# mmp/pbrt-v1

Hardware: AMD Instinct MI355X
Metric: Mrays/s (primary+secondary: every Scene::Intersect + Scene::IntersectP) (higher is better)
Workload: dtype f32

## Files before the change

pbrt-v1_amd/csrc/hip/rt_integrate.h:

```cpp
#pragma once
#include "rt_shade.h"
#include "rt_texture.h"
#include "rt_fixed_frame.h"
#include "rt_ray_guard.h"

namespace rt {

enum Stage {
    ST_FETCH = 0, ST_VERTEX, ST_DIRECT_NEXT, ST_SHADOW_DONE, ST_MIS_DONE, ST_ED_BSDF, ST_ED_DONE,
    ST_BOUNCE, ST_SPECULAR, ST_SPEC_TRANS, ST_RETURN, ST_VOL_BEGIN, ST_VOL_STEP, ST_POP, ST_FINISH, ST_EXIT
};

struct Rng {
    uint32_t base, ctr;
    RT_DEV float next_float() { return rng_f32(base, ctr++); }
    RT_DEV uint32_t next_u32() { return rng_u32(base, ctr++); }
};

#define RT_FRAME_WORDS 25

struct Lane {
    uint32_t sample_index;
    uint32_t work;
    float image_x, image_y;
// ... 358 lines not shown
    }
    const int nx = sc.dens_n[0], ny = sc.dens_n[1], nz = sc.dens_n[2];
    const float voxx = (q.x - v.p0[0]) / (v.p1[0] - v.p0[0]) * float(nx) - .5f;
    const float voxy = (q.y - v.p0[1]) / (v.p1[1] - v.p0[1]) * float(ny) - .5f;
    const float voxz = (q.z - v.p0[2]) / (v.p1[2] - v.p0[2]) * float(nz) - .5f;
    const int vx = int(floorf(voxx)), vy = int(floorf(voxy)), vz = int(floorf(voxz));
    const float dx = voxx - float(vx), dy = voxy - float(vy), dz = voxz - float(vz);
    const int x0 = clamp_ref(vx, 0, nx - 1), x1 = clamp_ref(vx + 1, 0, nx - 1);
    const int y0 = clamp_ref(vy, 0, ny - 1), y1 = clamp_ref(vy + 1, 0, ny - 1);
    const int z0 = clamp_ref(vz, 0, nz - 1), z1 = clamp_ref(vz + 1, 0, nz - 1);
    const float RT_G *g = RT_GPTR(const float, sc.dens_grid);
    const int r00 = z0 * nx * ny + y0 * nx, r10 = z0 * nx * ny + y1 * nx, r01 = z1 * nx * ny + y0 * nx, r11 = z1 * nx * ny + y1 * nx;
    const float c000 = g[r00 + x0], c100 = g[r00 + x1], c010 = g[r10 + x0], c110 = g[r10 + x1];
    const float c001 = g[r01 + x0], c101 = g[r01 + x1], c011 = g[r11 + x0], c111 = g[r11 + x1];
    const float d00 = lerp_ref(dx, c000, c100), d10 = lerp_ref(dx, c010, c110);
    const float d01 = lerp_ref(dx, c001, c101), d11 = lerp_ref(dx, c011, c111);
    const float d0 = lerp_ref(dy, d00, d10), d1 = lerp_ref(dy, d01, d11);
    return lerp_ref(dz, d0, d1);
}
RT_DEV V3 density_tau(const DevScene &sc, const DevFrame &fr, V3 o, V3 d, float mint, float maxt, float step, float u) {
    const float length = len3(d);
    if (length == 0.f) return mk3(0.f);
    const float inv = 1.f / length;
    const V3 dn = mk3(d.x * inv, d.y * inv, d.z * inv);
    float t0, t1;
    if (!vol_intersect(sc.vol, o, dn, mint * length, maxt * length, t0, t1)) return mk3(0.f);
    const V3 sig_t = mat_color(sc.vol.sigma_a) + mat_color(sc.vol.sigma_s);
    V3 tau = mk3(0.f);
    t0 += u * step;
    const int cap = fr.dens_cap;
#pragma unroll 1
    for (int k = 0; t0 < t1 && k < cap; ++k) {
        const float D = density_at(sc, xform_point(sc.vol.world_to_volume, o + dn * t0));
        tau = tau + sig_t * D;
        t0 += step;
    }
    return tau * step;
}
RT_DEV V3 exp_neg(V3 tau) { return mk3(rt_expf(-tau.x), rt_expf(-tau.y), rt_expf(-tau.z)); }

template <bool VOL, bool EXT>
RT_DEV V3 scene_transmittance(const DevScene &sc, const DevFrame &fr, Lane &ln, V3 o, V3 d, float mint, float maxt) {
    if (!VOL) return mk3(1.f);
    const float u = ln.rng.next_float();
    if (EXT && sc.dens_kind != RT_DENSITY_NONE) return exp_neg(density_tau(sc, fr, o, d, mint, maxt, 4.f * fr.step_size, u));
    return vol_transmittance(sc.vol, o, d, mint, maxt);
}

template <class SX>
RT_DEV decltype(auto) light_of(const DevScene &sc, int i) {
    if constexpr (SX::one_light) return (RT_LIGHT_K(sc));
    else return (RT_LIGHT(sc, i));
}
template <class SX>
RT_DEV DimReq light_dim(const DevFrame &fr, int li, int k) {
    if constexpr (SX::one_light) { const DimReq r = RT_KPTR(const DimReq, fr.light_dims)[k]; return r; }
    else { const DimReq r = (RT_GPTR(const DimReq, fr.light_dims) + 3 * li)[k]; return r; }
}
template <bool EXT, bool DEFER = false, bool GEOM_N = false, class SX = fixed::AnyScene, int ACCEL = -1>
RT_DEV void estimate_direct_bsdf(const DevScene &sc, Lane &ln) {
    const auto &Lt = light_of<SX>(sc, ln.cur_light);
    ln.stage = ST_ED_DONE;
    if (light_is_delta<EXT>(Lt)) return;
    MatRef m = RT_MAT(sc, ln.v.mat);
    V3 wi; float bsdfPdf; int sampled;
    V3 f = bsdf_sample_f<EXT>(m, ln.v, ln.v.wo, wi, ln.bs1, ln.bs2, ln.bcs, bsdfPdf, BX_ALL & ~BX_SPECULAR, sampled);
    if (!is_black(f) && bsdfPdf > 0.f) {
        float lightPdf;
        if constexpr (EXT) lightPdf = light_is_infinite<EXT>(Lt) ? infinite_pdf_cosine(GEOM_N ? ln.v.ng : ln.v.nn, wi) : area_light_pdf<EXT, SX::one_light>(sc, Lt, ln.v.p, wi);
        else lightPdf = area_light_pdf<EXT, SX::one_light>(sc, Lt, ln.v.p, wi);
        if (lightPdf > 0.f) {
            float fw = 1 * bsdfPdf, gw = 1 * lightPdf;
            float weight = (fw * fw) / (fw * fw + gw * gw);
            ln.pend = div_s(((f * mat_color(Lt.color)) * absdot3(wi, GEOM_N ? ln.v.ng : ln.v.nn)) * weight, bsdfPdf);
            launch_ray<DEFER, ACCEL>(ln, sc, ln.v.p, wi, RT_RAY_EPSILON, RT_INF, false, ST_MIS_DONE);
        }
    }
}

RT_DEV bool light_draws_rng(LightRef L) { return L.type == RT_LIGHT_AREA && L.quadric < 0 && L.n_tris > 1u; }
RT_DEV size_t weighted_record(const DevFrame &fr, const Lane &ln, int nLights) {
    if (!fr.wt_mixed) return size_t(ln.ord) * size_t(1 + 2 * nLights);
    const size_t j = ln.ord - RT_GPTR(const unsigned, fr.wt_base)[ln.work];
    return size_t(RT_GPTR(const unsigned, fr.wt_recbase)[ln.work]) + j * size_t(1 + 2 * (nLights - int(fr.wt_nd))) + size_t(fr.wt_nd) * j * (j + 1);
}

template <bool EXT, bool DEFER = false, bool GEOM_N = false, class SX = fixed::AnyScene, int ACCEL = -1>
RT_DEV void estimate_direct_begin(const DevScene &sc, Lane &ln, int light, float ls1, float ls2) {
    ln.cur_light = light;
    ln.Ld = mk3(0.f);
    const auto &Lt = light_of<SX>(sc, light);
    MatRef m = RT_MAT(sc, ln.v.mat);
    V3 wi, Li, sd; float lightPdf, smax;
    if (light_is_delta<EXT>(Lt)) {
        Li = delta_light_sample(Lt, ln.v.p, wi, sd, smax);
        lightPdf = 1.f;
    } else if constexpr (EXT) {
        if (light_is_infinite<EXT>(Lt)) {
            wi = infinite_sample_cosine(GEOM_N ? ln.v.ng : ln.v.nn, ls1, ls2, ln.rng, lightPdf);
            Li = mat_color(Lt.color);
            sd = wi; smax = RT_INF;
        } else {
            V3 ns;
            V3 ps = area_sample_point<EXT, SX::one_light>(sc, Lt, ln.v.p, ls1, ls2, ln.rng, ns);
            wi = normalize3(ps - ln.v.p);
            lightPdf = area_light_pdf<EXT, SX::one_light>(sc, Lt, ln.v.p, wi);
            Li = area_L(Lt, ns, -wi);
            sd = ps - ln.v.p; smax = 1.f - RT_RAY_EPSILON;
        }
    } else {
        V3 ns;
        V3 ps = area_sample_point<EXT, SX::one_light>(sc, Lt, ln.v.p, ls1, ls2, ln.rng, ns);
        wi = normalize3(ps - ln.v.p);
        lightPdf = area_light_pdf<EXT, SX::one_light>(sc, Lt, ln.v.p, wi);
        Li = area_L(Lt, ns, -wi);
        sd = ps - ln.v.p; smax = 1.f - RT_RAY_EPSILON;
    }
    if (lightPdf > 0.f && !is_black(Li)) {
        V3 f = bsdf_f<EXT>(m, ln.v, ln.v.wo, wi);
        if (!is_black(f)) {
            if (light_is_delta<EXT>(Lt)) ln.pend = div_s((f * Li) * absdot3(wi, GEOM_N ? ln.v.ng : ln.v.nn), lightPdf);
            else {
                float bsdfPdf = bsdf_pdf<EXT>(m, ln.v, ln.v.wo, wi);
                float fw = 1 * lightPdf, gw = 1 * bsdfPdf;
                float weight = (fw * fw) / (fw * fw + gw * gw);
                ln.pend = div_s(((f * Li) * absdot3(wi, GEOM_N ? ln.v.ng : ln.v.nn)) * weight, lightPdf);
            }
            launch_ray<DEFER, ACCEL>(ln, sc, ln.v.p, sd, RT_RAY_EPSILON, smax, true, ST_SHADOW_DONE);
            return;
        }
    }
    ln.stage = ST_ED_BSDF;
}

struct March { int i, N; float t0, step; V3 Tr, p, Lv; float s0, s1, s2; };
template <bool EXT>
RT_DEV void march_begin(const DevScene &sc, const DevFrame &fr, Lane &ln, const Ray &ray, March &m, float RT_G *samp, size_t st) {
    const RtVolume &vol = sc.vol;
    const bool single = fr.volume_integrator == RT_VOLUME_SINGLE;
    int N; float t0, t1, step; V3 p;
    if (!vol_intersect(vol, ray.o, ray.d, ray.mint, ray.maxt, t0, t1) || (t1 - t0) == 0.f) { N = 0; step = 0.f; p = ray.o; }
    else {
        N = int(ceilf((t1 - t0) / fr.step_size));
        step = (t1 - t0) / N;
        p = ray.o + ray.d * t0;
        t0 += dim_value(fr, ln, fr.one_d[fr.n1d - 1], 0, 0) * step;
        if (single) {
            if (N > fr.vol_nmax) { N = fr.vol_nmax; }
            const float delta = 1.f / N;
            for (int a = 0; a < N; ++a) for (int b = 0; b < 3; ++b) samp[size_t(3 * a + b) * st] = (a + ln.rng.next_float()) * delta;
            for (int b = 0; b < 3; ++b) for (int a = 0; a < N; ++a) {
                const int other = int(ln.rng.next_u32() % uint32_t(N));
                const float tmp = samp[size_t(3 * a + b) * st]; samp[size_t(3 * a + b) * st] = samp[size_t(3 * other + b) * st]; samp[size_t(3 * other + b) * st] = tmp;
            }
        }
    }
    m.i = 0; m.N = N; m.t0 = t0; m.step = step; m.Tr = mk3(1.f); m.p = p; m.Lv = mk3(0.f);
    if (EXT && sc.dens_kind != RT_DENSITY_NONE) {
        const V3 T = exp_neg(density_tau(sc, fr, ray.o, ray.d, ray.mint, ray.maxt, fr.step_size, dim_value(fr, ln, fr.one_d[fr.n1d - 2], 0, 0)));
        ln.L = T * ln.L;
    }
}
template <bool COUNT, bool EXT, bool DEFER, bool PREFETCH = false>
RT_DEV bool march_steps(const DevScene &sc, const DevFrame &fr, Lane &ln, const Ray &ray, March &m, const float RT_G *samp, size_t st, bool resume, unsigned *c_any) {
    const RtVolume &vol = sc.vol;
    const bool single = fr.volume_integrator == RT_VOLUME_SINGLE;
    int i = m.i; const int N = m.N; float t0 = m.t0; const float step = m.step; V3 Tr = m.Tr, p = m.p, Lv = m.Lv;
    const V3 w = -ray.d;
    bool have_row = false;
    if (resume) {
        if (COUNT) ++*c_any;
        if (ln.tv.hit_prim < 0)
            Lv = Lv + ln.pend * scene_transmittance<true, EXT>(sc, fr, ln, ln.tv.o, ln.tv.d, ln.tv.mint, ln.tv.maxt);
        ++i; t0 += step;
        have_row = PREFETCH;
    }
// ... 287 lines not shown
        const int nLights = SX::one_light ? 1 : int(sc.n_lights);
        if constexpr (WEIGHTED) {
            if (fr.weighted_phase == 2) {
                const unsigned at = fr.wt_mixed ? __float_as_uint(ln.wt_w) : 1u + 2u * unsigned(ln.li);
                float RT_G *rec = RT_GPTR(float, fr.wt_rec) + weighted_record(fr, ln, nLights) + at;
                rec[0] = lum_y(ln.Ld);
                rec[1] = lum_y(ln.Ld * float(nLights));
                if (fr.wt_mixed) {
                    ln.wt_w = __uint_as_float(at + 2u);
                    const unsigned j = ln.ord - RT_GPTR(const unsigned, fr.wt_base)[ln.work];
                    if (light_draws_rng(RT_LIGHT(sc, ln.li)) && unsigned(ln.lj) < j) ++ln.lj; else { ln.lj = 0; ++ln.li; }
                } else ++ln.li;
                ln.stage = ST_DIRECT_NEXT;
            } else {
                if (ln.wt_w == 0.f) ln.L = ln.L + ln.Ld * float(nLights);
                else ln.L = ln.L + div_s(ln.Ld, ln.wt_w);
                ln.stage = ST_SPECULAR;
            }
            return;
        }
        if (INTEG == RT_INTEGRATOR_PATH) {
            ln.L = ln.L + ln.thr * (ln.Ld * float(nLights));
            ln.stage = ST_BOUNCE;
        } else if (fr.strategy == RT_STRATEGY_ONE) {
            ln.L = ln.L + ln.Ld * float(nLights);
            ln.stage = ST_SPECULAR;
        } else {
            ln.Ld_light = ln.Ld_light + ln.Ld;
            if constexpr (SX::one_light && FX::all_n1) {
                ln.L_all = ln.L_all + ln.Ld_light * (1.f / float(1));
                ln.lj = 0; ln.li = 1;
                all_lights_done(ln);
                return;
            }
            const int ns = FX::all_n1 ? 1 : SX::one_light ? int(RT_KPTR(const DimReq, fr.light_dims)[0].n) : int(RT_GPTR(const DimReq, fr.light_dims)[3 * ln.li].n);
            if (++ln.lj >= ns) {
                ln.L_all = ln.L_all + ln.Ld_light * (1.f / float(ns));
                ln.lj = 0; ++ln.li;
            }
            ln.stage = ST_DIRECT_NEXT;
            if (ln.li >= nLights) all_lights_done(ln);
        }
        return;
    }
    if constexpr (STAGE == ST_BOUNCE) {
        MatRef m = RT_MAT(sc, ln.v.mat);
        const int k = ln.depth;
        float bs1, bs2, bcs;
        if (k < 3) {
            bs1 = dim_value<FX>(fr, ln, fr.two_d[3 * k + 2], 0, 0); bs2 = dim_value<FX>(fr, ln, fr.two_d[3 * k + 2], 0, 1);
            bcs = dim_value<FX>(fr, ln, fr.one_d[3 * k + 2], 0, 0);
        } else { bs1 = ln.rng.next_float(); bs2 = ln.rng.next_float(); bcs = ln.rng.next_float(); }
        V3 wi; float pdf; int flags;
        V3 f = bsdf_sample_f<EXT>(m, ln.v, ln.v.wo, wi, bs1, bs2, bcs, pdf, BX_ALL, flags);
        if (is_black(f) || pdf == 0.f) { ln.stage = ST_RETURN; return; }
        ln.specular = !SX::no_specular && (flags & BX_SPECULAR) != 0;
        ln.thr = ln.thr * div_s(f * absdot3(wi, ln.v.nn), pdf);
        if (k > 3) {
            if (ln.rng.next_float() > .5f) { ln.stage = ST_RETURN; return; }
            ln.thr = div_s(ln.thr, .5f);
        }
        if (k == fr.max_depth) { ln.stage = ST_RETURN; return; }
        ++ln.depth;
        launch_ray<DEFER, ACCEL>(ln, sc, ln.v.p, wi, RT_RAY_EPSILON, RT_INF, false, ST_VERTEX);
        return;
    }
    if constexpr (STAGE == ST_SPECULAR && SX::no_specular) {
        if (!(ln.depth < fr.max_depth)) { ln.stage = ST_RETURN; return; }
        ln.rng.ctr += 3u;
        ln.stage = ST_SPEC_TRANS;
        return;
    } else if constexpr (STAGE == ST_SPEC_TRANS && SX::no_specular) {
        ln.rng.ctr += 3u;
        ln.stage = ST_RETURN;
        return;
    } else if constexpr (STAGE == ST_POP && SX::no_specular && !VOL) {
        ln.stage = ST_FINISH;
        return;
    }
    if constexpr (STAGE == ST_SPECULAR) {
        if (!(ln.depth < fr.max_depth)) { ln.stage = ST_RETURN; return; }
        MatRef m = RT_MAT(sc, ln.v.mat);
        float u3 = ln.rng.next_float(), u2 = ln.rng.next_float(), u1 = ln.rng.next_float();
        V3 wi; float pdf; int flags;
        V3 f = bsdf_sample_f<EXT>(m, ln.v, ln.v.wo, wi, u1, u2, u3, pdf, BX_REFLECTION | BX_SPECULAR, flags);
        if (!is_black(f) && pdf > 0.f) f = div_s(f, pdf);
        const float ad = absdot3(wi, ln.v.nn);
        if (!is_black(f) && ad > 0.f) {
            frame_push<EXT>(fr, ln, gtid, f, ad, ST_SPEC_TRANS);
            ++ln.depth;
            launch_ray<DEFER, ACCEL>(ln, sc, ln.v.p, wi, RT_RAY_EPSILON, RT_INF, false, ST_VERTEX);
            if (VOL) { Ray cr; cr.o = ln.v.p; cr.d = wi; cr.mint = RT_RAY_EPSILON; cr.maxt = RT_INF; vol_store_ray(fr, ln.fsp, gtid, cr); }
            return;
        }
        ln.stage = ST_SPEC_TRANS;
        return;
    }
    if constexpr (STAGE == ST_SPEC_TRANS) {
        MatRef m = RT_MAT(sc, ln.v.mat);
        float u3 = ln.rng.next_float(), u2 = ln.rng.next_float(), u1 = ln.rng.next_float();
        V3 wi; float pdf; int flags;
        V3 f = bsdf_sample_f<EXT>(m, ln.v, ln.v.wo, wi, u1, u2, u3, pdf, BX_TRANSMISSION | BX_SPECULAR, flags);
        if (!is_black(f) && pdf > 0.f) f = div_s(f, pdf);
        const float ad = absdot3(wi, ln.v.nn);
        if (!is_black(f) && ad > 0.f) {
            frame_push<EXT>(fr, ln, gtid, f, ad, ST_RETURN);
            ++ln.depth;
// ... 176 lines not shown
```

pbrt-v1_amd/csrc/hip/rt_shade.h:

```cpp
#pragma once
#include "rt_traverse.h"

namespace rt {

enum { BX_REFLECTION = 1, BX_TRANSMISSION = 2, BX_DIFFUSE = 4, BX_GLOSSY = 8, BX_SPECULAR = 16,
       BX_ALL = 31 };

struct Vertex {
    V3 p, nn, sn, tn;
    V3 ng;
    V3 wo;
    int mat, light;
};

RT_DEV void tri_frame(V3 p1, V3 p2, V3 p3, bool flip, V3 &nn, V3 &dpdu) {
    const float du1 = 0.f - 1.f, du2 = 1.f - 1.f, dv1 = 0.f - 1.f, dv2 = 0.f - 1.f;
    V3 dp1 = p1 - p3, dp2 = p2 - p3;
    const float determinant = du1 * dv2 - dv1 * du2;
    const float invdet = 1.f / determinant;
    dpdu = (dv2 * dp1 - dv1 * dp2) * invdet;
    V3 dpdv = (-du2 * dp1 + du1 * dp2) * invdet;
    nn = normalize3(cross3(dpdu, dpdv));
    if (flip) nn = nn * -1.f;
}
// ... 236 lines not shown
    return p;
}
RT_DEV float diffuse_pdf(V3 wo, V3 wi) { return (wo.z * wi.z > 0.f) ? fabsf(wi.z) * RT_INV_PI : 0.f; }
RT_DEV float glossy_pdf(MatRef m, V3 wo, V3 wi) { return (wo.z * wi.z > 0.f) ? blinn_pdf(m.exponent, wo, wi) : 0.f; }
RT_DEV float diffuse_t_pdf(V3 wo, V3 wi) { return diffuse_pdf(wo, -wi); }
RT_DEV float glossy_t_pdf(MatRef m, V3 wo, V3 wi) { return glossy_pdf(m, wo, -wi); }

template <bool EXT> RT_DEV bool mat_has_diffuse(MatRef m) { return m.type == RT_MAT_MATTE || (EXT && (m.type == RT_MAT_PLASTIC || ((m.type == RT_MAT_UBER || m.type == RT_MAT_TRANSLUCENT) && m.has_r))); }
template <bool EXT> RT_DEV bool mat_has_glossy(MatRef m) { return EXT && (m.type == RT_MAT_PLASTIC || m.type == RT_MAT_SHINYMETAL || ((m.type == RT_MAT_UBER || m.type == RT_MAT_TRANSLUCENT) && m.has_g)); }
template <bool EXT> RT_DEV bool mat_has_diffuse_t(MatRef m) { return EXT && m.type == RT_MAT_TRANSLUCENT && m.has_t; }
template <bool EXT> RT_DEV bool mat_has_glossy_t(MatRef m) { return EXT && m.type == RT_MAT_TRANSLUCENT && m.has_kr; }
RT_DEV bool flags_match(int type, int flags) { return (type & flags) == type; }

template <bool EXT>
RT_DEV int bsdf_num_components(MatRef m, int flags) {
    int n = 0;
    if (EXT && m.type == RT_MAT_UBER) {
        if (m.has_t && flags_match(BX_TRANSMISSION | BX_SPECULAR, flags)) ++n;
        if (m.has_r && flags_match(BX_REFLECTION | BX_DIFFUSE, flags)) ++n;
        if (m.has_g && flags_match(BX_REFLECTION | BX_GLOSSY, flags)) ++n;
        if (m.has_kr && flags_match(BX_REFLECTION | BX_SPECULAR, flags)) ++n;
        return n;
    }
    if (EXT && m.type == RT_MAT_SHINYMETAL) return int(flags_match(BX_REFLECTION | BX_GLOSSY, flags)) + int(flags_match(BX_REFLECTION | BX_SPECULAR, flags));
    if (EXT && m.type == RT_MAT_TRANSLUCENT) {
        if (m.has_r && flags_match(BX_REFLECTION | BX_DIFFUSE, flags)) ++n;
        if (m.has_t && flags_match(BX_TRANSMISSION | BX_DIFFUSE, flags)) ++n;
        if (m.has_g && flags_match(BX_REFLECTION | BX_GLOSSY, flags)) ++n;
        if (m.has_kr && flags_match(BX_TRANSMISSION | BX_GLOSSY, flags)) ++n;
        return n;
    }
    if (m.type == RT_MAT_MATTE || (EXT && m.type == RT_MAT_PLASTIC)) {
        if (((BX_REFLECTION | BX_DIFFUSE) & flags) == (BX_REFLECTION | BX_DIFFUSE)) ++n;
        if (EXT && m.type == RT_MAT_PLASTIC && ((BX_REFLECTION | BX_GLOSSY) & flags) == (BX_REFLECTION | BX_GLOSSY)) ++n;
    } else {
        if (m.has_r && ((BX_REFLECTION | BX_SPECULAR) & flags) == (BX_REFLECTION | BX_SPECULAR)) ++n;
        if (m.type == RT_MAT_GLASS && m.has_t && ((BX_TRANSMISSION | BX_SPECULAR) & flags) == (BX_TRANSMISSION | BX_SPECULAR)) ++n;
    }
    return n;
}
template <bool EXT> RT_DEV int bsdf_total_components(MatRef m) { return bsdf_num_components<EXT>(m, BX_ALL); }

template <bool EXT>
RT_DEV V3 bsdf_f_lobes(MatRef m, V3 wo, V3 wi, int flags) {
    V3 f = mk3(0.f);
    if (mat_has_diffuse<EXT>(m) && flags_match(BX_REFLECTION | BX_DIFFUSE, flags)) f = f + diffuse_f(m, wo, wi);
    if (mat_has_diffuse_t<EXT>(m) && flags_match(BX_TRANSMISSION | BX_DIFFUSE, flags)) f = f + diffuse_t_f(m);
    if (mat_has_glossy<EXT>(m) && flags_match(BX_REFLECTION | BX_GLOSSY, flags)) f = f + microfacet_f(m, wo, wi);
    if (mat_has_glossy_t<EXT>(m) && flags_match(BX_TRANSMISSION | BX_GLOSSY, flags)) f = f + microfacet_t_f(m, wo, wi);
    return f;
}
template <bool EXT> RT_DEV bool mat_has_btdf(MatRef m) { return mat_has_diffuse_t<EXT>(m) || mat_has_glossy_t<EXT>(m); }

template <bool EXT>
RT_DEV V3 bsdf_f(MatRef m, const Vertex &v, V3 woW, V3 wiW) {
    if (!mat_has_diffuse<EXT>(m) && !mat_has_glossy<EXT>(m) && !mat_has_btdf<EXT>(m)) return mk3(0.f);
    V3 wi = to_local(v, wiW), wo = to_local(v, woW);
    if (dot3(wiW, vertex_ng<EXT>(v)) * dot3(woW, vertex_ng<EXT>(v)) > 0) return bsdf_f_lobes<EXT>(m, wo, wi, BX_ALL & ~BX_TRANSMISSION);
    if (mat_has_btdf<EXT>(m)) return bsdf_f_lobes<EXT>(m, wo, wi, BX_ALL & ~BX_REFLECTION);
    return mk3(0.f);
}

template <bool EXT>
RT_DEV float bsdf_pdf(MatRef m, const Vertex &v, V3 woW, V3 wiW) {
    int nc = bsdf_total_components<EXT>(m);
    if (nc == 0) return 0.f;
    if (!mat_has_diffuse<EXT>(m) && !mat_has_glossy<EXT>(m) && !mat_has_btdf<EXT>(m)) return 0.f / float(nc);
    V3 wo = to_local(v, woW), wi = to_local(v, wiW);
    float pdf = 0.f;
    if (mat_has_diffuse<EXT>(m)) pdf += diffuse_pdf(wo, wi);
    if (mat_has_diffuse_t<EXT>(m)) pdf += diffuse_t_pdf(wo, wi);
    if (mat_has_glossy<EXT>(m)) pdf += glossy_pdf(m, wo, wi);
    if (mat_has_glossy_t<EXT>(m)) pdf += glossy_t_pdf(m, wo, wi);
    return pdf / nc;
}

template <bool EXT>
RT_DEV V3 bsdf_f_flags(MatRef m, const Vertex &v, V3 woW, V3 wiW, int flags) {
    const V3 wi = to_local(v, wiW), wo = to_local(v, woW);
    if (dot3(wiW, vertex_ng<EXT>(v)) * dot3(woW, vertex_ng<EXT>(v)) > 0) flags &= ~BX_TRANSMISSION;
    else flags &= ~BX_REFLECTION;
    return bsdf_f_lobes<EXT>(m, wo, wi, flags);
}
template <bool EXT>
RT_DEV float bsdf_pdf_flags(MatRef m, const Vertex &v, V3 woW, V3 wiW, int flags) {
    const int nc = bsdf_num_components<EXT>(m, flags);
    if (nc == 0) return 0.f;
    const V3 wo = to_local(v, woW), wi = to_local(v, wiW);
    float pdf = 0.f;
    if (mat_has_diffuse<EXT>(m) && flags_match(BX_REFLECTION | BX_DIFFUSE, flags)) pdf += diffuse_pdf(wo, wi);
    if (mat_has_diffuse_t<EXT>(m) && flags_match(BX_TRANSMISSION | BX_DIFFUSE, flags)) pdf += diffuse_t_pdf(wo, wi);
    if (mat_has_glossy<EXT>(m) && flags_match(BX_REFLECTION | BX_GLOSSY, flags)) pdf += glossy_pdf(m, wo, wi);
    if (mat_has_glossy_t<EXT>(m) && flags_match(BX_TRANSMISSION | BX_GLOSSY, flags)) pdf += glossy_t_pdf(m, wo, wi);
    return pdf / nc;
}

template <bool EXT>
RT_DEV V3 bsdf_sample_f(MatRef m, const Vertex &v, V3 woW, V3 &wiW, float u1, float u2, float u3,
                        float &pdf, int flags, int &sampled) {
    sampled = 0; pdf = 0.f;
    int matching = bsdf_num_components<EXT>(m, flags);
    if (matching == 0) return mk3(0.f);
    int which = min(int(floorf(u3 * matching)), matching - 1);
    V3 wo = to_local(v, woW);
    V3 wi, f;
    const bool diffuse_has = mat_has_diffuse<EXT>(m) && flags_match(BX_REFLECTION | BX_DIFFUSE, flags);
    const bool glossy_has = mat_has_glossy<EXT>(m) && flags_match(BX_REFLECTION | BX_GLOSSY, flags);
    const bool diffuse_t_has = mat_has_diffuse_t<EXT>(m) && flags_match(BX_TRANSMISSION | BX_DIFFUSE, flags);
    const bool glossy_t_has = mat_has_glossy_t<EXT>(m) && flags_match(BX_TRANSMISSION | BX_GLOSSY, flags);
    const bool shiny = EXT && m.type == RT_MAT_SHINYMETAL;
    int pick = 0;
    if (shiny) {
        int idx = which;
        if (glossy_has && idx-- == 0) pick = 2;
        else if (flags_match(BX_REFLECTION | BX_SPECULAR, flags)) pick = 3;
    } else if (EXT && m.type == RT_MAT_TRANSLUCENT) {
        int idx = which;
        if (diffuse_has && idx-- == 0) pick = 1;
        else if (diffuse_t_has && idx-- == 0) pick = 5;
        else if (glossy_has && idx-- == 0) pick = 2;
        else if (glossy_t_has) pick = 6;
    } else if (EXT && m.type == RT_MAT_UBER) {
        int idx = which;
        const bool mT = m.has_t && flags_match(BX_TRANSMISSION | BX_SPECULAR, flags), mR = m.has_kr && flags_match(BX_REFLECTION | BX_SPECULAR, flags);
        if (mT && idx-- == 0) pick = 4;
        else if (diffuse_has && idx-- == 0) pick = 1;
        else if (glossy_has && idx-- == 0) pick = 2;
        else if (mR) pick = 3;
    } else if (diffuse_has || glossy_has) pick = (!glossy_has || (diffuse_has && which == 0)) ? 1 : 2;
    if (pick == 1 || pick == 2 || (EXT && (pick == 5 || pick == 6))) {
        const bool through = EXT && (pick == 5 || pick == 6);
        if (pick == 1 || (EXT && pick == 5)) {
            float dx, dy; concentric_disk(u1, u2, dx, dy);
            wi = mk3(dx, dy, sqrtf(fmaxf(0.f, 1.f - dx * dx - dy * dy)));
            if (wo.z < 0.f) wi.z *= -1.f;
            pdf = diffuse_pdf(wo, wi);
            if (pdf == 0.f) return mk3(0.f);
            sampled = through ? (BX_TRANSMISSION | BX_DIFFUSE) : (BX_REFLECTION | BX_DIFFUSE);
            if (through) wi = other_hemisphere(wi);
            if (through && diffuse_has) pdf += diffuse_pdf(wo, wi);
            if (!through && diffuse_t_has) pdf += diffuse_t_pdf(wo, wi);
            if (glossy_has) pdf += glossy_pdf(m, wo, wi);
            if (glossy_t_has) pdf += glossy_t_pdf(m, wo, wi);
        } else {
            const float costheta = rt_powf(u1, 1.f / (m.exponent + 1));
            const float sintheta = sqrtf(fmaxf(0.f, 1.f - costheta * costheta));
            const float phi = u2 * 2.f * RT_PI;
            V3 H = mk3(sintheta * rt_cosf(phi), sintheta * rt_sinf(phi), costheta);
            if (!(wo.z * H.z > 0.f)) H = -H;
            wi = -wo + H * (2.f * dot3(wo, H));
            pdf = ((m.exponent + 1.f) * rt_powf(costheta, m.exponent)) / (2.f * RT_PI * 4.f * dot3(wo, H));
            if (dot3(wo, H) <= 0.f) pdf = 0.f;
            if (pdf == 0.f) return mk3(0.f);
// ... 3 lines not shown
            if (diffuse_t_has) pdf += diffuse_t_pdf(wo, wi);
            if (through && glossy_has) pdf += glossy_pdf(m, wo, wi);
            if (!through && glossy_t_has) pdf += glossy_t_pdf(m, wo, wi);
        }
        wiW = to_world(v, wi);
        if (matching > 1) pdf /= matching;
        f = mk3(0.f);
        if (dot3(wiW, vertex_ng<EXT>(v)) * dot3(woW, vertex_ng<EXT>(v)) > 0) f = bsdf_f_lobes<EXT>(m, wo, wi, flags & ~BX_TRANSMISSION);
        else if (mat_has_btdf<EXT>(m)) f = bsdf_f_lobes<EXT>(m, wo, wi, flags & ~BX_REFLECTION);
        return f;
    }
    bool reflect_has = m.has_r && ((BX_REFLECTION | BX_SPECULAR) & flags) == (BX_REFLECTION | BX_SPECULAR);
    bool pick_reflect = ((EXT && m.type == RT_MAT_UBER) || shiny) ? pick == 3 : (reflect_has && which == 0);
    if (pick_reflect) {
        wi = mk3(-wo.x, -wo.y, wo.z);
        pdf = 1.f;
        const bool uber = EXT && m.type == RT_MAT_UBER;
        float F = (m.type == RT_MAT_GLASS) ? fresnel_dielectric(wo.z, 1.f, m.ior) : (uber ? fresnel_dielectric(wo.z, 1.5f, 1.f) : 1.f);
        if (shiny) f = div_s(fr_cond(fabsf(wo.z), mat_color(m.kr)) * mk3(1.f), fabsf(wi.z));
        else f = div_s(mk3(F) * (uber ? mat_color(m.kr) : mat_color(m.r)), fabsf(wi.z));
        sampled = BX_REFLECTION | BX_SPECULAR;
    } else {
        bool entering = wo.z > 0.f;
        float ei = 1.f, et = m.ior;
        if (!entering) { float tmp = ei; ei = et; et = tmp; }
        float sini2 = sin_theta2(wo);
        float eta = ei / et;
        float sint2 = eta * eta * sini2;
        if (sint2 >= 1.f) return mk3(0.f);
        float cost = sqrtf(fmaxf(0.f, 1.f - sint2));
        if (entering) cost = -cost;
        wi = mk3(eta * -wo.x, eta * -wo.y, cost);
        pdf = 1.f;
        float F = fresnel_dielectric(wo.z, 1.f, m.ior);
        f = div_s(((mk3(1.f) - mk3(F)) * ((et * et) / (ei * ei))) * mat_color(m.t), fabsf(wi.z));
        sampled = BX_TRANSMISSION | BX_SPECULAR;
    }
    wiW = to_world(v, wi);
    if (matching > 1) pdf /= matching;
    return f;
}

template <bool K = false>
RT_DEV void light_tri(const DevScene &sc, unsigned k, V3 &p1, V3 &p2, V3 &p3) {
    if constexpr (K) {
        const float RT_K *t = RT_KPTR(const float, sc.light_tris) + size_t(k) * 16;
        p1 = mk3(t[0], t[1], t[2]); p2 = mk3(t[3], t[4], t[5]); p3 = mk3(t[6], t[7], t[8]);
    } else {
    const float RT_G *t = RT_GPTR(const float, sc.light_tris) + size_t(k) * 16;
    p1 = mk3(t[0], t[1], t[2]); p2 = mk3(t[3], t[4], t[5]); p3 = mk3(t[6], t[7], t[8]);
    }
}

template <bool EXT, class LT> RT_DEV bool light_is_infinite(const LT &Lt) { return EXT && Lt.type == RT_LIGHT_INFINITE; }
template <bool EXT, class LT> RT_DEV bool light_is_delta(const LT &Lt) {
    if constexpr (EXT) return Lt.type != RT_LIGHT_AREA && Lt.type != RT_LIGHT_INFINITE;
    else return Lt.type != RT_LIGHT_AREA;
}
template <class LT>
RT_DEV V3 delta_light_sample(const LT &Lt, V3 p, V3 &wi, V3 &sd, float &smax) {
    if (Lt.type == RT_LIGHT_DISTANT) {
        wi = mk3(Lt.dir[0], Lt.dir[1], Lt.dir[2]);
        sd = wi; smax = RT_INF;
        return mat_color(Lt.color);
    }
    const V3 lp = mat_color(Lt.pos);
    const V3 dd = lp - p;
    wi = normalize3(dd);
    sd = dd; smax = 1.f - RT_RAY_EPSILON;
    const float d2 = dd.x * dd.x + dd.y * dd.y + dd.z * dd.z;
    if (Lt.type == RT_LIGHT_POINT) return div_s(mat_color(Lt.color), d2);
    const V3 w = -wi;
    const V3 wl = normalize3(mk3(Lt.w2l[0] * w.x + Lt.w2l[1] * w.y + Lt.w2l[2] * w.z, Lt.w2l[3] * w.x + Lt.w2l[4] * w.y + Lt.w2l[5] * w.z,
                                 Lt.w2l[6] * w.x + Lt.w2l[7] * w.y + Lt.w2l[8] * w.z));
    const float costheta = wl.z;
    float fall;
    if (costheta < Lt.cos_total) fall = 0.f;
    else if (costheta > Lt.cos_falloff) fall = 1.f;
    else { const float delta = (costheta - Lt.cos_total) / (Lt.cos_falloff - Lt.cos_total); fall = delta * delta * delta * delta; }
    return div_s(mat_color(Lt.color) * fall, d2);
}

RT_DEV void coordinate_system(V3 v1, V3 &v2, V3 &v3) {
    if (fabsf(v1.x) > fabsf(v1.y)) { const float il = 1.f / sqrtf(v1.x * v1.x + v1.z * v1.z); v2 = mk3(-v1.z * il, 0.f, v1.x * il); }
    else { const float il = 1.f / sqrtf(v1.y * v1.y + v1.z * v1.z); v2 = mk3(0.f, v1.z * il, -v1.y * il); }
    v3 = cross3(v1, v2);
}
template <class RNG>
RT_DEV V3 infinite_sample_cosine(V3 n, float u1, float u2, RNG &rng, float &pdf) {
    float x, y; concentric_disk(u1, u2, x, y);
    float z = sqrtf(fmaxf(0.f, 1.f - x * x - y * y));
    if (rng.next_float() < .5f) z *= -1.f;
    pdf = fabsf(z) * RT_INV_TWOPI;
    V3 v1, v2; coordinate_system(normalize3(n), v1, v2);
    return mk3(v1.x * x + v2.x * y + n.x * z, v1.y * x + v2.y * y + n.y * z, v1.z * x + v2.z * y + n.z * z);
}
RT_DEV float infinite_pdf_cosine(V3 n, V3 wi) { return absdot3(n, wi) * RT_INV_TWOPI; }
RT_DEV V3 infinite_sample_sphere(float u1, float u2, float &pdf) {
    const float z = 1.f - 2.f * u1;
    const float r = sqrtf(fmaxf(0.f, 1.f - z * z));
    const float phi = 2.f * RT_PI * u2;
    pdf = 1.f / (4.f * RT_PI);
    return mk3(r * rt_cosf(phi), r * rt_sinf(phi), z);
}
RT_DEV V3 infinite_le_sum(const DevScene &sc, V3 acc, V3 w, bool weighted) {
    if (sc.n_infinite == 0) return acc;
// ... 25 lines not shown
        const float r = sqrtf(fmaxf(0.f, 1.f - z * z));
        const float phi = 2.f * RT_PI * u2;
        p = mk3(0.f) + mk3(r * rt_cosf(phi), r * rt_sinf(phi), z) * q.radius;
        n = p;
    }
    ns = normalize3(xform_normal(q.w2o, n));
    if (ro) ns = ns * -1.f;
    return xform_point(q.o2w, p);
}
RT_DEV V3 quadric_sample(const DevScene &sc, unsigned qi, bool ro, V3 p, float u1, float u2, V3 &ns) {
    const DevQuadric RT_G &q = RT_GPTR(const DevQuadric, sc.quadrics)[qi];
    if (q.type != RT_QUADRIC_SPHERE) return quadric_sample_uniform(q, ro, u1, u2, ns);
    const V3 Pcenter = xform_point(q.o2w, mk3(0.f));
    const V3 wc = normalize3(Pcenter - p);
    V3 wcX, wcY;
    if (fabsf(wc.x) > fabsf(wc.y)) { const float il = 1.f / sqrtf(wc.x * wc.x + wc.z * wc.z); wcX = mk3(-wc.z * il, 0.f, wc.x * il); }
    else { const float il = 1.f / sqrtf(wc.y * wc.y + wc.z * wc.z); wcX = mk3(0.f, wc.z * il, -wc.y * il); }
    wcY = cross3(wc, wcX);
    if (dist_sq(p, Pcenter) - q.radius * q.radius < 1e-4f) return quadric_sample_uniform(q, ro, u1, u2, ns);
    const float cosThetaMax = sqrtf(fmaxf(0.f, 1.f - q.radius * q.radius / dist_sq(p, Pcenter)));
    const float costheta = (1.f - u1) * cosThetaMax + u1 * 1.f;
    const float sintheta = sqrtf(1.f - costheta * costheta);
    const float phi = u2 * 2.f * RT_PI;
    const V3 rd = wcX * (rt_cosf(phi) * sintheta) + wcY * (rt_sinf(phi) * sintheta) + wc * costheta;
    float thit;
    if (!quadric_test(sc, qi, p, rd, RT_RAY_EPSILON, RT_INF, thit)) thit = dot3(Pcenter - p, normalize3(rd));
    const V3 ps = p + rd * thit;
    ns = normalize3(ps - Pcenter);
    if (ro) ns = ns * -1.f;
    return ps;
}
RT_DEV float quadric_area(const DevQuadric RT_G &q) {
    return q.type == RT_QUADRIC_DISK ? q.phi_max * 0.5f * (q.radius * q.radius - q.zmax * q.zmax)
                                     : (q.type == RT_QUADRIC_CYLINDER ? (q.zmax - q.zmin) * q.phi_max * q.radius : q.phi_max * q.radius * (q.zmax - q.zmin));
}
RT_DEV float quadric_light_pdf(const DevScene &sc, unsigned qi, V3 p, V3 wi) {
    const DevQuadric RT_G &q = RT_GPTR(const DevQuadric, sc.quadrics)[qi];
    if (q.type == RT_QUADRIC_SPHERE) {
        const V3 Pcenter = xform_point(q.o2w, mk3(0.f));
        if (!(dist_sq(p, Pcenter) - q.radius * q.radius < 1e-4f)) {
            const float cosThetaMax = sqrtf(fmaxf(0.f, 1.f - q.radius * q.radius / dist_sq(p, Pcenter)));
            return 1.f / (2.f * RT_PI * (1.f - cosThetaMax));
        }
    }
    float thit;
    if (!quadric_test(sc, qi, p, wi, RT_RAY_EPSILON, RT_INF, thit)) return 0.f;
    V3 hp, nn, sn; quadric_frame(sc, qi, false, p, wi, thit, hp, nn, sn);
    const float area = quadric_area(q);
    float pdf = dist_sq(p, p + wi * thit) / (absdot3(nn, -wi) * area);
    if (absdot3(nn, -wi) == 0.f) pdf = 0.f;
    return pdf;
}

template <bool EXT, bool K = false, class LT>
RT_DEV float area_light_pdf(const DevScene &sc, const LT &L, V3 p, V3 wi) {
    if (EXT && L.quadric >= 0) return quadric_light_pdf(sc, unsigned(L.quadric), p, wi);
    bool any = false; float thit = 0.f; V3 nl = mk3(0.f);
    for (unsigned k = 0; k < L.n_tris; ++k) {
        V3 p1, p2, p3; light_tri<K>(sc, L.first_tri + k, p1, p2, p3);
        float t, b1, b2;
        if (tri_test(p1, p2 - p1, p3 - p1, p, wi, RT_RAY_EPSILON, RT_INF, t, b1, b2)) {
            any = true; thit = t;
            if constexpr (K) {
                const float RT_K *ltr = RT_KPTR(const float, sc.light_tris) + size_t(L.first_tri + k) * 16;
                nl = mk3(ltr[12], ltr[13], ltr[14]);
            } else {
            const float RT_G *ltr = RT_GPTR(const float, sc.light_tris) + size_t(L.first_tri + k) * 16;
            nl = mk3(ltr[12], ltr[13], ltr[14]);
            }
        }
    }
    if (!any) return 0.f;
    V3 ph = p + wi * thit;
    V3 dd = p - ph;
    float ad = absdot3(nl, -wi);
    float pdf = (dd.x * dd.x + dd.y * dd.y + dd.z * dd.z) / (ad * L.area);
    if (ad == 0.f) pdf = 0.f;
    return pdf;
}

template <class LT> RT_DEV V3 area_L(const LT &L, V3 n, V3 w) { return dot3(n, w) > 0 ? mat_color(L.color) : mk3(0.f); }

template <bool EXT, bool K = false, class LT, class RNG>
RT_DEV V3 area_sample_point(const DevScene &sc, const LT &L, V3 pref, float u1, float u2, RNG &rng, V3 &ns) {
    if (EXT && L.quadric >= 0) return quadric_sample(sc, unsigned(L.quadric), L.reverse_orientation != 0, pref, u1, u2, ns);
    unsigned k = 0;
    if (L.n_tris > 1) {
        float ls = rng.next_float();
        for (k = 0; k < L.n_tris - 1; ++k) {
            if constexpr (K) { if (ls < RT_KPTR(const float, sc.light_tris)[size_t(L.first_tri + k) * 16 + 10]) break; }
            else
            if (ls < RT_GPTR(const float, sc.light_tris)[size_t(L.first_tri + k) * 16 + 10]) break;
        }
    }
    V3 p1, p2, p3; light_tri<K>(sc, L.first_tri + k, p1, p2, p3);
    float su1 = sqrtf(u1);
    float b1 = 1.f - su1, b2 = u2 * su1;
    V3 ps = b1 * p1 + b2 * p2 + (1.f - b1 - b2) * p3;
    ns = normalize3(cross3(p2 - p1, p3 - p1));
    if (L.reverse_orientation) ns = ns * -1.f;
    return ps;
}

RT_DEV V3 uniform_sample_cone(float u1, float u2, float costhetamax) {
    const float costheta = (1.f - u1) * costhetamax + u1 * 1.f;
    const float sintheta = sqrtf(1.f - costheta * costheta);
    const float phi = u2 * 2.f * RT_PI;
    return mk3(rt_cosf(phi) * sintheta, rt_sinf(phi) * sintheta, costheta);
}
RT_DEV V3 light_to_world(LightRef Lt, V3 v) {
    const float inv = Lt.l2w_scale;
    return mk3((Lt.l2w[0] * v.x + Lt.l2w[1] * v.y + Lt.l2w[2] * v.z) * inv, (Lt.l2w[3] * v.x + Lt.l2w[4] * v.y + Lt.l2w[5] * v.z) * inv,
               (Lt.l2w[6] * v.x + Lt.l2w[7] * v.y + Lt.l2w[8] * v.z) * inv);
}
template <bool EXT, class RNG>
RT_DEV void light_sample_emission(const DevScene &sc, LightRef Lt, V3 wc, float wr, float u1, float u2, float u3, float u4, RNG &rng, V3 &o, V3 &d, float &pdf) {
    if (Lt.type == RT_LIGHT_POINT) {
        o = mat_color(Lt.pos);
        d = infinite_sample_sphere(u1, u2, pdf);
    } else if (Lt.type == RT_LIGHT_SPOT) {
        o = mat_color(Lt.pos);
        d = light_to_world(Lt, uniform_sample_cone(u1, u2, Lt.cos_total));
        pdf = 1.f / (2.f * RT_PI * (1.f - Lt.cos_total));
    } else if (Lt.type == RT_LIGHT_DISTANT) {
        const V3 lightDir = mat_color(Lt.dir);
        V3 v1, v2; coordinate_system(lightDir, v1, v2);
        float d1, d2; concentric_disk(u1, u2, d1, d2);
        const V3 Pdisk = wc + wr * (d1 * v1 + d2 * v2);
        o = Pdisk + wr * lightDir;
        d = -lightDir;
        pdf = 1.f / (RT_PI * wr * wr);
    } else if (Lt.type == RT_LIGHT_INFINITE) {
        const float worldRadius = wr * 1.01f;
        float unused;
        const V3 p1 = wc + worldRadius * infinite_sample_sphere(u1, u2, unused);
        const V3 p2 = wc + worldRadius * infinite_sample_sphere(u3, u4, unused);
        o = p1;
        d = normalize3(p2 - p1);
// ... 22 lines not shown
```

Baseline: 3686.

## Specialize direct lighting for single small emitters and matte-only scenes

Adds a fast path for scenes with one light and at most two emitter triangles. Both triangles are loaded from constant memory once and reused for area sampling and the pdf, instead of looping over triangle indices. It also copies the light header into registers and adds a diffuse-only BSDF path (f, pdf, sample) for scenes known to have no specular materials. This cuts redundant loads and lobe dispatch in the shading stage, but raises register pressure and adds more template code paths.

New measurement: 3755 (median of 6 runs). 1.02x the previous value.

```diff
diff --git a/pbrt-v1_amd/csrc/hip/rt_integrate.h b/pbrt-v1_amd/csrc/hip/rt_integrate.h
--- a/pbrt-v1_amd/csrc/hip/rt_integrate.h
+++ b/pbrt-v1_amd/csrc/hip/rt_integrate.h
@@ -434,6 +434,19 @@
     if constexpr (SX::one_light) return (RT_LIGHT_K(sc));
     else return (RT_LIGHT(sc, i));
 }
+#ifndef RT_EMITTER_HOIST
+#define RT_EMITTER_HOIST 1
+#endif
+struct LightHead { int type; float color[3]; unsigned first_tri, n_tris; int reverse_orientation; float area; int quadric; };
+template <class SX, class LT>
+RT_DEV decltype(auto) light_head(const LT &L) {
+    if constexpr (SX::one_light && RT_EMITTER_HOIST != 0) {
+        LightHead h;
+        h.type = L.type; h.color[0] = L.color[0]; h.color[1] = L.color[1]; h.color[2] = L.color[2];
+        h.first_tri = L.first_tri; h.n_tris = L.n_tris; h.reverse_orientation = L.reverse_orientation; h.area = L.area; h.quadric = L.quadric;
+        return h;
+    } else return (L);
+}
 template <class SX>
 RT_DEV DimReq light_dim(const DevFrame &fr, int li, int k) {
     if constexpr (SX::one_light) { const DimReq r = RT_KPTR(const DimReq, fr.light_dims)[k]; return r; }
@@ -441,12 +454,13 @@
 }
 template <bool EXT, bool DEFER = false, bool GEOM_N = false, class SX = fixed::AnyScene, int ACCEL = -1>
 RT_DEV void estimate_direct_bsdf(const DevScene &sc, Lane &ln) {
-    const auto &Lt = light_of<SX>(sc, ln.cur_light);
+    const auto &Ld = light_of<SX>(sc, ln.cur_light);
+    const auto &Lt = light_head<SX>(Ld);
     ln.stage = ST_ED_DONE;
     if (light_is_delta<EXT>(Lt)) return;
     MatRef m = RT_MAT(sc, ln.v.mat);
     V3 wi; float bsdfPdf; int sampled;
-    V3 f = bsdf_sample_f<EXT>(m, ln.v, ln.v.wo, wi, ln.bs1, ln.bs2, ln.bcs, bsdfPdf, BX_ALL & ~BX_SPECULAR, sampled);
+    V3 f = bsdf_sample_f<EXT, SX::no_specular>(m, ln.v, ln.v.wo, wi, ln.bs1, ln.bs2, ln.bcs, bsdfPdf, BX_ALL & ~BX_SPECULAR, sampled);
     if (!is_black(f) && bsdfPdf > 0.f) {
         float lightPdf;
         if constexpr (EXT) lightPdf = light_is_infinite<EXT>(Lt) ? infinite_pdf_cosine(GEOM_N ? ln.v.ng : ln.v.nn, wi) : area_light_pdf<EXT, SX::one_light>(sc, Lt, ln.v.p, wi);
@@ -471,11 +485,12 @@
 RT_DEV void estimate_direct_begin(const DevScene &sc, Lane &ln, int light, float ls1, float ls2) {
     ln.cur_light = light;
     ln.Ld = mk3(0.f);
-    const auto &Lt = light_of<SX>(sc, light);
+    const auto &Ld = light_of<SX>(sc, light);
+    const auto &Lt = light_head<SX>(Ld);
     MatRef m = RT_MAT(sc, ln.v.mat);
     V3 wi, Li, sd; float lightPdf, smax;
     if (light_is_delta<EXT>(Lt)) {
-        Li = delta_light_sample(Lt, ln.v.p, wi, sd, smax);
+        Li = delta_light_sample(Ld, ln.v.p, wi, sd, smax);
         lightPdf = 1.f;
     } else if constexpr (EXT) {
         if (light_is_infinite<EXT>(Lt)) {
@@ -490,6 +505,20 @@
             Li = area_L(Lt, ns, -wi);
             sd = ps - ln.v.p; smax = 1.f - RT_RAY_EPSILON;
         }
+    } else if constexpr (SX::one_light && RT_SMALL_EMITTER != 0) {
+        V3 ns, ps;
+        if (emitter_is_small(Lt)) {
+            const EmitterPair e = emitter_pair(sc, Lt);
+            ps = area_sample_point_small(e, Lt, ls1, ls2, ln.rng, ns);
+            wi = normalize3(ps - ln.v.p);
+            lightPdf = area_light_pdf_small(e, Lt, ln.v.p, wi);
+        } else {
+            ps = area_sample_point<EXT, true, false>(sc, Lt, ln.v.p, ls1, ls2, ln.rng, ns);
+            wi = normalize3(ps - ln.v.p);
+            lightPdf = area_light_pdf<EXT, true, false>(sc, Lt, ln.v.p, wi);
+        }
+        Li = area_L(Lt, ns, -wi);
+        sd = ps - ln.v.p; smax = 1.f - RT_RAY_EPSILON;
     } else {
         V3 ns;
         V3 ps = area_sample_point<EXT, SX::one_light>(sc, Lt, ln.v.p, ls1, ls2, ln.rng, ns);
@@ -499,11 +528,11 @@
         sd = ps - ln.v.p; smax = 1.f - RT_RAY_EPSILON;
     }
     if (lightPdf > 0.f && !is_black(Li)) {
-        V3 f = bsdf_f<EXT>(m, ln.v, ln.v.wo, wi);
+        V3 f = bsdf_f<EXT, SX::no_specular>(m, ln.v, ln.v.wo, wi);
         if (!is_black(f)) {
             if (light_is_delta<EXT>(Lt)) ln.pend = div_s((f * Li) * absdot3(wi, GEOM_N ? ln.v.ng : ln.v.nn), lightPdf);
             else {
-                float bsdfPdf = bsdf_pdf<EXT>(m, ln.v, ln.v.wo, wi);
+                float bsdfPdf = bsdf_pdf<EXT, SX::no_specular>(m, ln.v, ln.v.wo, wi);
                 float fw = 1 * lightPdf, gw = 1 * bsdfPdf;
                 float weight = (fw * fw) / (fw * fw + gw * gw);
                 ln.pend = div_s(((f * Li) * absdot3(wi, GEOM_N ? ln.v.ng : ln.v.nn)) * weight, lightPdf);
@@ -897,7 +926,7 @@
             bcs = dim_value<FX>(fr, ln, fr.one_d[3 * k + 2], 0, 0);
         } else { bs1 = ln.rng.next_float(); bs2 = ln.rng.next_float(); bcs = ln.rng.next_float(); }
         V3 wi; float pdf; int flags;
-        V3 f = bsdf_sample_f<EXT>(m, ln.v, ln.v.wo, wi, bs1, bs2, bcs, pdf, BX_ALL, flags);
+        V3 f = bsdf_sample_f<EXT, SX::no_specular>(m, ln.v, ln.v.wo, wi, bs1, bs2, bcs, pdf, BX_ALL, flags);
         if (is_black(f) || pdf == 0.f) { ln.stage = ST_RETURN; return; }
         ln.specular = !SX::no_specular && (flags & BX_SPECULAR) != 0;
         ln.thr = ln.thr * div_s(f * absdot3(wi, ln.v.nn), pdf);
diff --git a/pbrt-v1_amd/csrc/hip/rt_shade.h b/pbrt-v1_amd/csrc/hip/rt_shade.h
--- a/pbrt-v1_amd/csrc/hip/rt_shade.h
+++ b/pbrt-v1_amd/csrc/hip/rt_shade.h
@@ -312,8 +312,16 @@
 }
 template <bool EXT> RT_DEV bool mat_has_btdf(MatRef m) { return mat_has_diffuse_t<EXT>(m) || mat_has_glossy_t<EXT>(m); }
 
-template <bool EXT>
+#ifndef RT_MATTE_LOBES
+#define RT_MATTE_LOBES 1
+#endif
+template <bool EXT, bool MATTE = false>
 RT_DEV V3 bsdf_f(MatRef m, const Vertex &v, V3 woW, V3 wiW) {
+    if constexpr (MATTE && !EXT && RT_MATTE_LOBES != 0) {
+        V3 wi = to_local(v, wiW), wo = to_local(v, woW);
+        if (dot3(wiW, vertex_ng<EXT>(v)) * dot3(woW, vertex_ng<EXT>(v)) > 0) return mk3(0.f) + diffuse_f(m, wo, wi);
+        return mk3(0.f);
+    }
     if (!mat_has_diffuse<EXT>(m) && !mat_has_glossy<EXT>(m) && !mat_has_btdf<EXT>(m)) return mk3(0.f);
     V3 wi = to_local(v, wiW), wo = to_local(v, woW);
     if (dot3(wiW, vertex_ng<EXT>(v)) * dot3(woW, vertex_ng<EXT>(v)) > 0) return bsdf_f_lobes<EXT>(m, wo, wi, BX_ALL & ~BX_TRANSMISSION);
@@ -321,8 +329,14 @@
     return mk3(0.f);
 }
 
-template <bool EXT>
+template <bool EXT, bool MATTE = false>
 RT_DEV float bsdf_pdf(MatRef m, const Vertex &v, V3 woW, V3 wiW) {
+    if constexpr (MATTE && !EXT && RT_MATTE_LOBES != 0) {
+        V3 wo = to_local(v, woW), wi = to_local(v, wiW);
+        float pdf = 0.f;
+        pdf += diffuse_pdf(wo, wi);
+        return pdf / 1;
+    }
     int nc = bsdf_total_components<EXT>(m);
     if (nc == 0) return 0.f;
     if (!mat_has_diffuse<EXT>(m) && !mat_has_glossy<EXT>(m) && !mat_has_btdf<EXT>(m)) return 0.f / float(nc);
@@ -355,10 +369,24 @@
     return pdf / nc;
 }
 
-template <bool EXT>
+template <bool EXT, bool MATTE = false>
 RT_DEV V3 bsdf_sample_f(MatRef m, const Vertex &v, V3 woW, V3 &wiW, float u1, float u2, float u3,
                         float &pdf, int flags, int &sampled) {
     sampled = 0; pdf = 0.f;
+    if constexpr (MATTE && !EXT && RT_MATTE_LOBES != 0) {
+        if (!flags_match(BX_REFLECTION | BX_DIFFUSE, flags)) return mk3(0.f);
+        V3 wo = to_local(v, woW);
+        float dx, dy; concentric_disk(u1, u2, dx, dy);
+        V3 wi = mk3(dx, dy, sqrtf(fmaxf(0.f, 1.f - dx * dx - dy * dy)));
+        if (wo.z < 0.f) wi.z *= -1.f;
+        pdf = diffuse_pdf(wo, wi);
+        if (pdf == 0.f) return mk3(0.f);
+        sampled = BX_REFLECTION | BX_DIFFUSE;
+        wiW = to_world(v, wi);
+        V3 f = mk3(0.f);
+        if (dot3(wiW, vertex_ng<EXT>(v)) * dot3(woW, vertex_ng<EXT>(v)) > 0) f = mk3(0.f) + diffuse_f(m, wo, wi);
+        return f;
+    }
     int matching = bsdf_num_components<EXT>(m, flags);
     if (matching == 0) return mk3(0.f);
     int which = min(int(floorf(u3 * matching)), matching - 1);
@@ -468,6 +496,27 @@
     }
 }
 
+#ifndef RT_SMALL_EMITTER
+#define RT_SMALL_EMITTER 1
+#endif
+struct EmitterTri { V3 p1, p2, p3, n; float cdf; };
+struct EmitterPair { EmitterTri t0, t1; };
+RT_DEV EmitterTri emitter_tri(const DevScene &sc, unsigned k) {
+    const float RT_K *t = RT_KPTR(const float, sc.light_tris) + size_t(k) * 16;
+    EmitterTri e;
+    e.p1 = mk3(t[0], t[1], t[2]); e.p2 = mk3(t[3], t[4], t[5]); e.p3 = mk3(t[6], t[7], t[8]);
+    e.cdf = t[10];
+    e.n = mk3(t[12], t[13], t[14]);
+    return e;
+}
+template <class LT> RT_DEV bool emitter_is_small(const LT &L) { return L.n_tris - 1u <= 1u; }
+template <class LT> RT_DEV EmitterPair emitter_pair(const DevScene &sc, const LT &L) {
+    EmitterPair e;
+    e.t0 = emitter_tri(sc, L.first_tri);
+    e.t1 = emitter_tri(sc, L.first_tri + (L.n_tris - 1u));
+    return e;
+}
+
 template <bool EXT, class LT> RT_DEV bool light_is_infinite(const LT &Lt) { return EXT && Lt.type == RT_LIGHT_INFINITE; }
 template <bool EXT, class LT> RT_DEV bool light_is_delta(const LT &Lt) {
     if constexpr (EXT) return Lt.type != RT_LIGHT_AREA && Lt.type != RT_LIGHT_INFINITE;
@@ -599,9 +648,28 @@
     return pdf;
 }
 
-template <bool EXT, bool K = false, class LT>
+template <class LT>
+RT_DEV float area_light_pdf_small(const EmitterPair &e, const LT &L, V3 p, V3 wi) {
+    bool any = false; float thit = 0.f; V3 nl = mk3(0.f);
+    float t, b1, b2;
+    if (tri_test(e.t0.p1, e.t0.p2 - e.t0.p1, e.t0.p3 - e.t0.p1, p, wi, RT_RAY_EPSILON, RT_INF, t, b1, b2)) { any = true; thit = t; nl = e.t0.n; }
+    if (L.n_tris > 1u) {
+        if (tri_test(e.t1.p1, e.t1.p2 - e.t1.p1, e.t1.p3 - e.t1.p1, p, wi, RT_RAY_EPSILON, RT_INF, t, b1, b2)) { any = true; thit = t; nl = e.t1.n; }
+    }
+    if (!any) return 0.f;
+    V3 ph = p + wi * thit;
+    V3 dd = p - ph;
+    float ad = absdot3(nl, -wi);
+    float pdf = (dd.x * dd.x + dd.y * dd.y + dd.z * dd.z) / (ad * L.area);
+    if (ad == 0.f) pdf = 0.f;
+    return pdf;
+}
+template <bool EXT, bool K = false, bool SMALL = true, class LT>
 RT_DEV float area_light_pdf(const DevScene &sc, const LT &L, V3 p, V3 wi) {
     if (EXT && L.quadric >= 0) return quadric_light_pdf(sc, unsigned(L.quadric), p, wi);
+    if constexpr (K && SMALL && RT_SMALL_EMITTER != 0) {
+        if (emitter_is_small(L)) return area_light_pdf_small(emitter_pair(sc, L), L, p, wi);
+    }
     bool any = false; float thit = 0.f; V3 nl = mk3(0.f);
     for (unsigned k = 0; k < L.n_tris; ++k) {
         V3 p1, p2, p3; light_tri<K>(sc, L.first_tri + k, p1, p2, p3);
@@ -628,9 +696,27 @@
 
 template <class LT> RT_DEV V3 area_L(const LT &L, V3 n, V3 w) { return dot3(n, w) > 0 ? mat_color(L.color) : mk3(0.f); }
 
-template <bool EXT, bool K = false, class LT, class RNG>
+template <class LT, class RNG>
+RT_DEV V3 area_sample_point_small(const EmitterPair &e, const LT &L, float u1, float u2, RNG &rng, V3 &ns) {
+    float ls = 0.f;
+    if (L.n_tris > 1u) ls = rng.next_float();
+    const bool first = !(L.n_tris > 1u) || ls < e.t0.cdf;
+    const V3 p1 = mk3(first ? e.t0.p1.x : e.t1.p1.x, first ? e.t0.p1.y : e.t1.p1.y, first ? e.t0.p1.z : e.t1.p1.z);
+    const V3 p2 = mk3(first ? e.t0.p2.x : e.t1.p2.x, first ? e.t0.p2.y : e.t1.p2.y, first ? e.t0.p2.z : e.t1.p2.z);
+    const V3 p3 = mk3(first ? e.t0.p3.x : e.t1.p3.x, first ? e.t0.p3.y : e.t1.p3.y, first ? e.t0.p3.z : e.t1.p3.z);
+    float su1 = sqrtf(u1);
+    float b1 = 1.f - su1, b2 = u2 * su1;
+    V3 ps = b1 * p1 + b2 * p2 + (1.f - b1 - b2) * p3;
+    ns = normalize3(cross3(p2 - p1, p3 - p1));
+    if (L.reverse_orientation) ns = ns * -1.f;
+    return ps;
+}
+template <bool EXT, bool K = false, bool SMALL = true, class LT, class RNG>
 RT_DEV V3 area_sample_point(const DevScene &sc, const LT &L, V3 pref, float u1, float u2, RNG &rng, V3 &ns) {
     if (EXT && L.quadric >= 0) return quadric_sample(sc, unsigned(L.quadric), L.reverse_orientation != 0, pref, u1, u2, ns);
+    if constexpr (K && SMALL && RT_SMALL_EMITTER != 0) {
+        if (emitter_is_small(L)) return area_sample_point_small(emitter_pair(sc, L), L, u1, u2, rng, ns);
+    }
     unsigned k = 0;
     if (L.n_tris > 1) {
         float ls = rng.next_float();
```
